# UncertainLab/Enlsip.jl

Hardware: NVIDIA B200
Metric: batched CNLS solves/s (n=6,m=128) (higher is better)
Workload: dtype f64

## Files before the change

### enlsip.jl_b200/csrc/enl_base.h

```cpp
#pragma once
#include <math.h>
#include <stdint.h>
#include <type_traits>

#if defined(__CUDACC__)
#define ENL_FN __device__
#define ENL_INL __device__ __forceinline__
#define ENL_NOINL __device__ __noinline__
#else
#define ENL_FN
#define ENL_INL inline
#define ENL_NOINL
#endif

namespace enl {

#if defined(__CUDA_ARCH__)
ENL_INL double mul_rn(double a, double b) { return __dmul_rn(a, b); }
ENL_INL double add_rn(double a, double b) { return __dadd_rn(a, b); }
ENL_INL double sub_rn(double a, double b) { return __dsub_rn(a, b); }
ENL_INL double fma_rn(double a, double b, double c) { return fma(a, b, c); }
ENL_INL double div_rn(double a, double b) { return __ddiv_rn(a, b); }
ENL_INL double sqrt_rn(double a) { return __dsqrt_rn(a); }
#else
// ... 48 lines not shown
    acc = fma_rn(acc, r, 1.0);
    int k1 = k >> 1;
    int k2 = k - k1;
    double res = mul_rn(mul_rn(acc, pow2i(k1)), pow2i(k2));
    if (x < -745.2) res = 0.0;
    if (x > 709.782712893384) res = INFINITY;
    return (x != x) ? x : res;
}

ENL_INL double det_tanh(double z) {
    double e = det_exp(mul_rn(2.0, z));
    return sub_rn(1.0, div_rn(2.0, add_rn(e, 1.0)));
}

#if defined(__CUDACC__)
template <int G_>
struct DevGroup {
    static constexpr int G = G_;
    unsigned mask;
    int lane;
    __device__ DevGroup() {
        int wl = threadIdx.x & 31;
        lane = wl & (G - 1);
        mask = (G == 32) ? 0xffffffffu : (((1u << G) - 1u) << (wl & ~(G - 1)));
    }
    __device__ __forceinline__ void sync() const {
        if (G > 1) __syncwarp(mask);
    }
    __device__ __forceinline__ double sum(double v) const {
#pragma unroll
        for (int o = G / 2; o > 0; o >>= 1) v += __shfl_xor_sync(mask, v, o, G);
        return v;
    }
    __device__ __forceinline__ double maxv(double v) const {
#pragma unroll
        for (int o = G / 2; o > 0; o >>= 1) v = fmax(v, __shfl_xor_sync(mask, v, o, G));
        return v;
    }
};
#endif

struct HostGroup {
    static constexpr int G = 1;
    int lane = 0;
    void sync() const {}
    double sum(double v) const { return v; }
    double maxv(double v) const { return v; }
};

#if defined(__CUDACC__)
extern __shared__ __align__(16) double enl_smem[];
using vref = int;
ENL_INL vref make_vref(double* p) { return (int)(p - enl_smem); }
ENL_INL vref make_vref(int* p) { return (int)(p - reinterpret_cast<int*>(enl_smem)); }
ENL_INL double& vderef_d(vref o) { return enl_smem[o]; }
ENL_INL int& vderef_i(vref o) { return reinterpret_cast<int*>(enl_smem)[o]; }
#else
using vref = void*;
ENL_INL vref make_vref(double* p) { return p; }
ENL_INL vref make_vref(int* p) { return p; }
#endif

template <int S>
struct SV {
#if defined(__CUDACC__)
    int p;
    ENL_INL double& operator[](int i) const { return enl_smem[p + i * S]; }
#else
    double* p;
    ENL_INL double& operator[](int i) const { return p[i * S]; }
#endif
    ENL_INL SV off(int k) const { return SV{p + k * S}; }
};
template <int S>
struct SI {
#if defined(__CUDACC__)
    int p;
    ENL_INL int& operator[](int i) const { return reinterpret_cast<int*>(enl_smem)[p + i * S]; }
#else
// ... 44 lines not shown
```

### enlsip.jl_b200/csrc/enl_linalg.h

```cpp
#pragma once
#include "enl_base.h"

namespace enl {

#if defined(ENL_HOST_BUILD)
typedef void (*host_dgeqp3_fn)(const int*, const int*, double*, const int*, int*, double*, double*, const int*, int*);
inline host_dgeqp3_fn& host_dgeqp3() { static host_dgeqp3_fn fn = nullptr; return fn; }
inline void host_lapack_qrcp(double* a, int ld, int rows, int cols, double* tau, int* jpvt) {
    static thread_local double work[8192];
    for (int j = 0; j < cols; ++j) jpvt[j] = 0;
    int info = 0;
    const int lwork = 8192;
    host_dgeqp3()(&rows, &cols, a, &ld, jpvt, tau, work, &lwork, &info);
    for (int j = 0; j < cols; ++j) jpvt[j] -= 1;
}
#endif

template <class V>
ENL_NOINL double nrm2_small(V a, int n) {
    double s = 0.0;
#pragma unroll 1
    for (int i = 0; i < n; ++i) s += a[i] * a[i];
    return sqrt(s);
}
// ... 124 lines not shown
        x[i] = s / d;
    }
    return true;
}

template <class V, class V2>
ENL_NOINL bool solve_upperT_small(V R, int ld, int k, V2 x) {
#pragma unroll 1
    for (int i = 0; i < k; ++i) {
        double s = x[i];
#pragma unroll 1
        for (int j = 0; j < i; ++j) s -= R[i * ld + j] * x[j];
        double d = R[i * ld + i];
        if (d == 0.0) return false;
        x[i] = s / d;
    }
    return true;
}

template <class V>
ENL_NOINL int pseudo_rank(V R, int ld, int len, double eps_rank) {
    if (len <= 0 || fabs(R[0]) < eps_rank) return 0;
    double tol = fabs(R[0]) * sqrt((double)len) * eps_rank;
    int r = 1;
#pragma unroll 1
    while (r < len && fabs(R[(r - 1) * ld + (r - 1)]) > tol) ++r;
    return r - ((r == len && fabs(R[(r - 1) * ld + (r - 1)]) > tol) ? 0 : 1);
}

template <class Grp, int G, int MS, int NT>
struct Dist {
    Grp g;

    ENL_NOINL double colsq(DM<G, MS, NT> a, int c, int r0) const {
        double s = 0.0;
#pragma unroll
        for (int sl = 0; sl < MS; ++sl) {
            int row = sl * G + g.lane;
            double v = a.at(sl, c);
            if (row >= r0) s += v * v;
        }
        return g.sum(s);
    }

    template <class V>
    ENL_NOINL void mul_q_right(DM<G, MS, NT> J, int n, V fa, int ld, int k, V tau) const {
#pragma unroll 1
        for (int i = 0; i < k; ++i) {
            double ti = tau[i];
            if (ti == 0.0) continue;
#pragma unroll
            for (int sl = 0; sl < MS; ++sl) {
                double wv = J.at(sl, i);
#pragma unroll 1
                for (int c = i + 1; c < n; ++c) wv += J.at(sl, c) * fa[i * ld + c];
                wv *= ti;
                J.at(sl, i) -= wv;
#pragma unroll 1
                for (int c = i + 1; c < n; ++c) J.at(sl, c) -= wv * fa[i * ld + c];
            }
        }
    }

    template <class V, class VI>
    ENL_NOINL void qrcp(DM<G, MS, NT> a, int M, int ncols, V tau2, VI jpvt, V vn1, V vn2, V Rout, int ldr) const {
#if defined(ENL_HOST_BUILD)
        if (host_dgeqp3() && G == 1 && NT == 1 && M > 0 && ncols > 0) {
            host_lapack_qrcp(&a.at(0, 0), MS, M, ncols, &tau2[0], &jpvt[0]);
            const int kk = imin(M, ncols);
            for (int c = 0; c < ncols; ++c)
                for (int r = 0; r < kk; ++r) Rout[c * ldr + r] = (r <= c) ? a.row(r, c) : 0.0;
            return;
        }
#endif
#pragma unroll 1
        for (int j = 0; j < ncols; ++j) {
            jpvt[j] = j;
            double nj = sqrt(colsq(a, j, 0));
            vn1[j] = nj;
            vn2[j] = nj;
        }
        int k = imin(M, ncols);
#pragma unroll 1
        for (int i = 0; i < k; ++i) {
            int pvt = i;
            double best = vn1[i];
#pragma unroll 1
            for (int j = i + 1; j < ncols; ++j)
                if (vn1[j] > best) { best = vn1[j]; pvt = j; }
            if (pvt != i) {
#pragma unroll
                for (int sl = 0; sl < MS; ++sl) {
                    double tmp = a.at(sl, pvt);
                    a.at(sl, pvt) = a.at(sl, i);
                    a.at(sl, i) = tmp;
                }
                int it = jpvt[pvt]; jpvt[pvt] = jpvt[i]; jpvt[i] = it;
                vn1[pvt] = vn1[i];
                vn2[pvt] = vn2[i];
            }
            g.sync();
            double tau_i = 0.0;
            if (i < M - 1) {
                double alpha = a.row(i, i);
                double xn = sqrt(colsq(a, i, i + 1));
                if (xn != 0.0) {
                    double beta = -sign_of(lapy2(alpha, xn), alpha);
                    tau_i = (beta - alpha) / beta;
                    double sc = 1.0 / (alpha - beta);
                    g.sync();
#pragma unroll
                    for (int sl = 0; sl < MS; ++sl) {
                        int row = sl * G + g.lane;
                        if (row > i) a.at(sl, i) *= sc;
                        else if (row == i) a.at(sl, i) = beta;
                    }
                }
            }
            tau2[i] = tau_i;
            if (i < ncols - 1 && tau_i != 0.0) {
#pragma unroll 1
                for (int c = i + 1; c < ncols; ++c) {
                    double part = 0.0;
#pragma unroll
                    for (int sl = 0; sl < MS; ++sl) {
                        int row = sl * G + g.lane;
                        double vv = (row > i) ? a.at(sl, i) : ((row == i) ? 1.0 : 0.0);
                        part += vv * a.at(sl, c);
                    }
                    double wv = g.sum(part) * tau_i;
#pragma unroll
                    for (int sl = 0; sl < MS; ++sl) {
                        int row = sl * G + g.lane;
                        if (row > i) a.at(sl, c) -= wv * a.at(sl, i);
                        else if (row == i) a.at(sl, c) -= wv;
                    }
                }
            }
            g.sync();
#pragma unroll 1
            for (int j = i + 1; j < ncols; ++j) {
                double v1 = vn1[j];
                if (v1 != 0.0) {
                    double tq = fabs(a.row(i, j)) / v1;
                    double temp = fmax(1.0 - tq * tq, 0.0);
                    double rq = v1 / vn2[j];
                    double temp2 = temp * (rq * rq);
                    if (temp2 <= TOL3Z) {
                        if (i < M - 1) {
                            double nj = sqrt(colsq(a, j, i + 1));
                            vn1[j] = nj;
                            vn2[j] = nj;
                        } else {
                            vn1[j] = 0.0;
                            vn2[j] = 0.0;
                        }
                    } else {
                        vn1[j] = v1 * sqrt(temp);
                    }
                }
            }
        }
        g.sync();
#pragma unroll 1
        for (int c = 0; c < ncols; ++c)
#pragma unroll 1
            for (int r = 0; r < k; ++r) Rout[c * ldr + r] = (r <= c) ? a.row(r, c) : 0.0;
    }

    template <class V>
// ... 13 lines not shown
#pragma unroll
            for (int sl = 0; sl < MS; ++sl) {
                int row = sl * G + g.lane;
                if (row > i) d.at(sl, 0) -= wv * a.at(sl, i);
                else if (row == i) d.at(sl, 0) -= wv;
            }
        }
        g.sync();
    }

    template <class V>
    ENL_NOINL void apply_q_regs(DM<G, MS, NT> a, int k, V tau2, double* v) const {
#pragma unroll 1
        for (int i = k - 1; i >= 0; --i) {
            double ti = tau2[i];
            if (ti == 0.0) continue;
            double part = 0.0;
#pragma unroll
            for (int sl = 0; sl < MS; ++sl) {
                int row = sl * G + g.lane;
                double vv = (row > i) ? a.at(sl, i) : ((row == i) ? 1.0 : 0.0);
                part += vv * v[sl];
            }
            double wv = g.sum(part) * ti;
#pragma unroll
            for (int sl = 0; sl < MS; ++sl) {
                int row = sl * G + g.lane;
                double vv = (row > i) ? a.at(sl, i) : ((row == i) ? 1.0 : 0.0);
                v[sl] -= wv * vv;
            }
        }
    }

    ENL_NOINL double prefix_sq(DM<G, MS, NT> d, int len) const {
        double s = 0.0;
#pragma unroll
        for (int sl = 0; sl < MS; ++sl) {
            int row = sl * G + g.lane;
            double v = d.at(sl, 0);
            if (row < len) s += v * v;
        }
        return g.sum(s);
    }
};

}
```

### enlsip.jl_b200/csrc/enl_solver.h

```cpp
#pragma once
#include "enl_base.h"
#include "enl_linalg.h"
#include "enl_families.h"

namespace enl {

struct Options {
    int max_iter;
    int scaling;
    int jac_mode;
    int second_derivatives;
    double time_limit;
    double eps_abs;
    double eps_rel;
    double eps_x;
    double eps_c;
    double eps_rank;
};

constexpr int MAX_N = 32;
struct Bounds {
    int nlo, nup;
    int lo_idx[MAX_N], up_idx[MAX_N];
    double lo_val[MAX_N], up_val[MAX_N];
// ... 24 lines not shown
    static constexpr size_t smem_bytes() {
        return (size_t)nD * PPC * 8 + (size_t)DCOLS * MS * NT * 8 + (size_t)nI * PPC * 4;
    }
};

struct IterRec {
    int t, rankA, rankJ2, dimA, dimJ2, code, index_del, index_alpha_upp, nb_newton;
    bool restart, add, del;
    double alpha, beta, progress, predicted_reduction, grad_res, speed;
};

struct Outputs {
    double* x;
    double* f;
    int* exit_code;
    int* status;
    int* iters;
    int* nact;
    int* active;
    int* counters;
    double* trace;
    int trace_cap;
};

template <class Fam, class Grp, int NT>
struct Solver {
    static constexpr int G = Grp::G;
    using LY = Layout<Fam, G, NT>;
    static constexpr int N = LY::N, M = LY::M, Q = LY::Q, NNL = LY::NNL, LMAX = LY::LMAX, T = LY::T, PPC = LY::PPC,
                         MS = LY::MS;
    using V = SV<PPC>;
    using VI = SI<PPC>;
    using D = DM<G, MS, NT>;

    V x, xprev, xnew, cx, cnew, A, gradf, w, wnew, K, acx, aA, dsc, FA, tauA, FL, tauL, R2, tau2, lam, b, p, y, Ap, aAp,
        v1c, vn1, vn2, s1, s2, s3, s4, s5, nw;
    VI active, inactive, permA, permL, perm2, posidx;
    D dR, dJ, dF, dD, dY;
    V fs;
    using FCtx = typename Fam::template Ctx<D, V>;
    ENL_INL Grp grp() const { return Grp(); }
    ENL_INL Dist<Grp, G, MS, NT> dst() const { return Dist<Grp, G, MS, NT>(); }
    ENL_INL FCtx fctx() const { return FCtx{dY, fs}; }
    const Options& opt;
    const Bounds& bnd;

    int l, t, k_iter, ndetail, exit_code;
    int n_res, n_cons, n_jres, n_jcons;
    bool threw, hang;
    bool j2_factored;
    IterRec cur, prev;
    double rx_sum, active_cx_sum, f_detail, rdot_x1, cdot_x1, rdot_prev, cdot_prev;
    double jp_r, jp_jp;
    double t_start;

    ENL_FN Solver(double* small, int* ints, double* distbase, int pid, const Options& o, const Bounds& bb)
        : opt(o), bnd(bb) {
#if defined(__CUDACC__)
        int s = (int)(small - enl_smem) + pid;
#else
        double* s = small + pid;
#endif
        auto mk = [&](int off) { return V{s + off * PPC}; };
        x = mk(LY::oX); xprev = mk(LY::oXPREV); xnew = mk(LY::oXNEW); cx = mk(LY::oCX); cnew = mk(LY::oCNEW);
        A = mk(LY::oA); gradf = mk(LY::oGRADF); w = mk(LY::oW); wnew = mk(LY::oWNEW); K = mk(LY::oK);
        acx = mk(LY::oACX); aA = mk(LY::oAA); dsc = mk(LY::oDSC); FA = mk(LY::oFA); tauA = mk(LY::oTAUA);
// ... 6 lines not shown
#else
        int* ii = ints + pid;
#endif
        auto mi = [&](int off) { return VI{ii + off * PPC}; };
        active = mi(LY::iACT); inactive = mi(LY::iINACT); permA = mi(LY::iPERMA); permL = mi(LY::iPERML);
        perm2 = mi(LY::iPERM2); posidx = mi(LY::iPOS);
#if defined(__CUDACC__)
        int grpb = (int)(distbase - enl_smem) + pid * G;
#else
        double* grpb = distbase + pid * G;
#endif
        D all{grpb};
        dR = all; dJ = all.cols(1); dF = dJ; dD = all.cols(1 + N); dY = all.cols(2 + N);
        l = NNL + bnd.nlo + bnd.nup;
    }

    ENL_FN void load_x(V src, double* xv) const {
#pragma unroll
        for (int j = 0; j < N; ++j) xv[j] = src[j];
    }

    ENL_NOINL void eval_point(const double* xv, double* rn, V cout) {
        Fam::template residuals<Grp, MS>(fctx(), grp(), xv, rn);
        double cnl[NNL > 0 ? NNL : 1];
        if (NNL > 0) Fam::template constraints<MS>(fctx(), xv, cnl);
#pragma unroll 1
        for (int i = 0; i < NNL; ++i) cout[i] = cnl[i];
#pragma unroll 1
        for (int j = 0; j < bnd.nlo; ++j) cout[NNL + j] = sub_rn(xv[bnd.lo_idx[j]], bnd.lo_val[j]);
#pragma unroll 1
        for (int j = 0; j < bnd.nup; ++j) cout[NNL + bnd.nlo + j] = sub_rn(bnd.up_val[j], xv[bnd.up_idx[j]]);
    }

    ENL_FN double sumsq_regs(const double* rn) const {
        double s = 0.0;
#pragma unroll
        for (int sl = 0; sl < MS; ++sl) s += rn[sl] * rn[sl];
        return grp().sum(s);
    }

    const double* mat_J = nullptr;
    ENL_NOINL void eval_res_jacobian() {
        if (mat_J) {
#pragma unroll
            for (int sl = 0; sl < MS; ++sl) {
                const int row = sl * G + grp().lane;
#pragma unroll
                for (int j = 0; j < N; ++j) dJ.at(sl, j) = (row < M) ? mat_J[(size_t)j * M + row] : 0.0;
            }
            j2_factored = false;
            grp().sync();
            return;
        }
        double xv[N];
        load_x(x, xv);
        double out[MS * N];
        if (opt.jac_mode == 0) {
            Fam::template jac_residuals<Grp, MS>(fctx(), grp(), xv, out);
        } else {
            double r0[MS], dl[N];
#pragma unroll
            for (int sl = 0; sl < MS; ++sl) r0[sl] = dR.at(sl, 0);
#pragma unroll
            for (int j = 0; j < N; ++j) dl[j] = mul_rn(fmax(fabs(xv[j]), 1.0), SQRT_EPS);
            fd_res(xv, r0, dl, out);
        }
// ... 35 lines not shown
            } else {
                double xf[N], cf[NNL > 0 ? NNL : 1];
#pragma unroll 1
                for (int j = 0; j < N; ++j) {
                    double dj = mul_rn(fmax(fabs(xv[j]), 1.0), SQRT_EPS);
#pragma unroll 1
                    for (int i = 0; i < N; ++i) xf[i] = xv[i];
                    xf[j] = add_rn(xv[j], dj);
                    Fam::template constraints<MS>(fctx(), xf, cf);
#pragma unroll 1
                    for (int i = 0; i < NNL; ++i) An[i * N + j] = div_z(sub_rn(cf[i], cx[i]), dj);
                }
            }
#pragma unroll 1
            for (int i = 0; i < NNL * N; ++i) A[i] = An[i];
        }
    }

    ENL_NOINL void init_bound_rows() {
#pragma unroll 1
        for (int j = 0; j < bnd.nlo; ++j)
#pragma unroll 1
            for (int c = 0; c < N; ++c) A[(NNL + j) * N + c] = (c == bnd.lo_idx[j]) ? 1.0 : 0.0;
#pragma unroll 1
        for (int j = 0; j < bnd.nup; ++j)
#pragma unroll 1
            for (int c = 0; c < N; ++c) A[(NNL + bnd.nlo + j) * N + c] = (c == bnd.up_idx[j]) ? -1.0 : 0.0;
    }

    ENL_NOINL void grad_and_sumsq() {
        double rr[MS];
#pragma unroll
        for (int sl = 0; sl < MS; ++sl) rr[sl] = dR.at(sl, 0);
#pragma unroll 1
        for (int j = 0; j < N; ++j) {
            double s = 0.0;
#pragma unroll
            for (int sl = 0; sl < MS; ++sl) s += dJ.at(sl, j) * rr[sl];
            gradf[j] = grp().sum(s);
        }
        rx_sum = sumsq_regs(rr);
    }

    ENL_FN void ws_remove(int s) {
        int lt = l - t;
        int id = active[s - 1];
        int pos = lt;
#pragma unroll 1
        while (pos > 0 && inactive[pos - 1] > id) { inactive[pos] = inactive[pos - 1]; --pos; }
        inactive[pos] = id;
#pragma unroll 1
        for (int i = s; i <= t - 1; ++i) active[i - 1] = active[i];
        active[t - 1] = 0;
        t -= 1;
    }
    ENL_FN void ws_add(int s) {
        int id = inactive[s - 1];
        int pos = t;
#pragma unroll 1
        while (pos > 0 && active[pos - 1] > id) { active[pos] = active[pos - 1]; --pos; }
        active[pos] = id;
#pragma unroll 1
        for (int i = s; i <= l - t - 1; ++i) inactive[i - 1] = inactive[i];
        inactive[l - t - 1] = 0;
        t += 1;
    }

    ENL_NOINL bool evaluate_violated_constraints(int index_alpha_upp) {
        const double delta = 0.1;
        int cap = imin(l, N);
        bool added = false;
        int swaps = 0;
        if (l > t) {
            int i = 1;
// ... 73 lines not shown
#pragma unroll 1
        for (int i = 0; i < N; ++i) s1[i] = gradf[i];
        apply_qt_small(FA, N, N, t, tauA, s1);
#pragma unroll 1
        for (int i = 0; i < t; ++i) s2[i] = (i < pr) ? s1[i] : 0.0;
        if (!solve_upper_small(FA, N, pr, s2)) threw = true;
        double gr = 0.0;
#pragma unroll 1
        for (int i = pr; i < N; ++i) gr += s1[i] * s1[i];
        cur.grad_res = (N > pr) ? sqrt(gr) : 0.0;
#pragma unroll 1
        for (int j = 0; j < t; ++j) s3[j] = (j < pr) ? -acx[permA[j]] : 0.0;
        if (!solve_upperT_small(FA, N, pr, s3)) threw = true;
        if (!solve_upper_small(FA, N, pr, s3)) threw = true;
#pragma unroll 1
        for (int j = 0; j < t; ++j) lam[permA[j]] = s2[j] + s3[j];
        if (opt.scaling)
#pragma unroll 1
            for (int i = 0; i < t; ++i) lam[i] = lam[i] * dsc[i];
    }

    ENL_NOINL void second_lagrange() {
        int pr = pseudo_rank(FA, N, t, SQRT_EPS);
        double v[MS];
        {
            const int kq = imin(M, N - cur.rankA);
#pragma unroll
            for (int sl = 0; sl < MS; ++sl) {
                int row = sl * G + grp().lane;
                v[sl] = (row >= kq) ? -dD.at(sl, 0) : 0.0;
            }
            dst().apply_q_regs(dF, kq, tau2, v);
        }
#pragma unroll 1
        for (int j = 0; j < t; ++j) {
            double s = 0.0;
#pragma unroll
            for (int sl = 0; sl < MS; ++sl) s += dJ.at(sl, j) * v[sl];
            s1[j] = grp().sum(s);
        }
#pragma unroll 1
        for (int j = pr; j < t; ++j) s1[j] = 0.0;
        if (!solve_upper_small(FA, N, pr, s1)) threw = true;
#pragma unroll 1
        for (int j = 0; j < t; ++j) lam[permA[j]] = s1[j];
        if (opt.scaling)
#pragma unroll 1
            for (int i = 0; i < t; ++i) lam[i] = lam[i] * dsc[i];
    }

    ENL_NOINL int check_constraint_deletion(double grad_res) {
        double lam_max = 1.0;
        if (t > 0) {
            lam_max = 0.0;
#pragma unroll 1
            for (int i = 0; i < t; ++i) lam_max = fmax(lam_max, fabs(lam[i]));
        }
        double sq_rel = SQRT_EPS * lam_max;
        int s = 0;
        if (t > Q) {
            double e = sq_rel;
#pragma unroll 1
            for (int i = Q + 1; i <= t; ++i) {
                double row_i = opt.scaling ? 1.0 / dsc[i - 1] : dsc[i - 1];
                double v = row_i * lam[i - 1];
                if (v <= sq_rel && v <= e) { e = v; s = i; }
            }
            if (grad_res > -e * 10.0) s = 0;
        }
        return s;
    }

    ENL_FN void minmax_lagrangian_mult(double& sigmin, double& lam_abs_max) {
// ... 3 lines not shown
#pragma unroll 1
            for (int i = 0; i < t; ++i) lam_abs_max = fmax(lam_abs_max, fabs(lam[i]));
#pragma unroll 1
            for (int i = Q; i < t; ++i) {
                double rows = opt.scaling ? 1.0 / dsc[i] : dsc[i];
                double li = lam[i];
                if (li * rows <= -SQRT_EPS && li < sigmin) sigmin = li;
            }
        }
    }

    ENL_NOINL void sub_search_direction(int rankA, int dimA, int dimJ2, int code) {
        const int k2 = N - rankA;
        const int kq = imin(M, k2);
        if (code == 1) {
#pragma unroll 1
            for (int j = 0; j < t; ++j) { double v = -acx[permA[j]]; b[j] = v; y[j] = v; }
            if (!solve_upperT_small(FA, N, t, y)) threw = true;
        } else {
#pragma unroll 1
            for (int j = 0; j < t; ++j) s1[j] = -acx[permA[j]];
            apply_qt_small(FL, T, t, t, tauL, s1);
#pragma unroll 1
            for (int j = 0; j < t; ++j) b[j] = s1[j];
            if (dimA > t || dimA < 0) { threw = true; dimA = imax(0, imin(dimA, t)); }
#pragma unroll 1
            for (int j = 0; j < t; ++j) s2[j] = (j < dimA) ? s1[j] : 0.0;
            if (!solve_upper_small(FL, T, dimA, s2)) threw = true;
#pragma unroll 1
            for (int j = 0; j < t; ++j) s3[permL[j]] = s2[j];
#pragma unroll 1
            for (int j = 0; j < rankA; ++j) y[j] = s3[j];
        }
#pragma unroll
        for (int sl = 0; sl < MS; ++sl) {
            double acc = 0.0;
#pragma unroll 1
            for (int c = 0; c < rankA; ++c) acc += dJ.at(sl, c) * y[c];
            dD.at(sl, 0) = -acc - dR.at(sl, 0);
        }
        grp().sync();
        dst().apply_qt(dF, kq, tau2, dD);
        if (dimJ2 > kq || dimJ2 < 0) { threw = true; dimJ2 = imax(0, imin(dimJ2, kq)); }
#pragma unroll 1
        for (int j = 0; j < dimJ2; ++j) s2[j] = dD.row(j, 0);
        if (!solve_upper_small(R2, N, dimJ2, s2)) threw = true;
#pragma unroll 1
        for (int j = 0; j < k2; ++j) y[rankA + perm2[j]] = (j < dimJ2) ? s2[j] : 0.0;
#pragma unroll 1
        for (int j = 0; j < N; ++j) p[j] = y[j];
        apply_q_small(FA, N, N, t, tauA, p);
    }

    ENL_NOINL void gn_search_direction(int rankA) {
        int code = (rankA == t) ? 1 : -1;
        dst().mul_q_right(dJ, N, FA, N, t, tauA);
        const int k2 = N - rankA;
        dF = dJ.cols(rankA);
        grp().sync();
        dst().qrcp(dF, M, k2, tau2, perm2, vn1, vn2, R2, N);
        j2_factored = true;
        int rankJ2 = pseudo_rank(R2, N, imin(M, k2), opt.eps_rank);
        sub_search_direction(rankA, rankA, rankJ2, code);
        cur.rankA = rankA;
        cur.rankJ2 = rankJ2;
        cur.dimA = rankA;
        cur.dimJ2 = rankJ2;
    }

    ENL_NOINL void update_working_set() {
        factor_A();
        first_lagrange();
        int s = check_constraint_deletion(cur.grad_res);
        if (s != 0) {
            cur.index_del = 0;
            cur.del = false;
            if (opt.scaling) {
#pragma unroll 1
                for (int i = 0; i < t; ++i) {
                    int id = active[i] - 1;
#pragma unroll 1
                    for (int c = 0; c < N; ++c) aA[i * N + c] = A[id * N + c] * dsc[i];
                }
                factor_A();
            }
        }
#pragma unroll 1
        for (int pass = 0; pass < 2; ++pass) {
            int rankA = pseudo_rank(FA, N, t, opt.eps_rank);
            factor_L11();
            gn_search_direction(rankA);
            if (pass == 0 && t == rankA && cur.rankJ2 == imin(M, N - rankA)) {
                second_lagrange();
// ... 102 lines not shown
        double prev_alpha = prev.alpha;
        int pdA;
        const int k2 = N - rankA;
        const int kq = imin(M, k2);
        if (rankA <= 0) {
            dimA = 0;
            pdA = 0;
#pragma unroll
            for (int sl = 0; sl < MS; ++sl) dD.at(sl, 0) = -dR.at(sl, 0);
        } else {
            pdA = abs(prev.dimA) + t - prev.t;
            if (pdA > t) { threw = true; pdA = t; }
            double sb = 0.0, sa = 0.0;
#pragma unroll 1
            for (int j = 0; j < t; ++j) {
                sb += b[j] * b[j];
                if (j < pdA) sa += b[j] * b[j];
            }
            double nrm_b = sqrt(sb), nrm_b_asprev = sqrt(sa);
            double cprog = cdot_prev - active_cx_sum;
            dimA = determine_solving_dim(pdA, rankA, nrm_b, cprog, nrm_b_asprev, FL, T, b, prev_alpha, restart);
            if (dimA > t || rankA - dimA < 0) { threw = true; dimA = imin(dimA, rankA); }
#pragma unroll 1
            for (int j = 0; j < rankA; ++j) s2[j] = (j < dimA) ? b[j] : 0.0;
            if (!solve_upper_small(FL, T, dimA, s2)) threw = true;
#pragma unroll 1
            for (int i = 0; i < rankA; ++i) {
                double acc = 0.0;
#pragma unroll 1
                for (int j = 0; j < rankA; ++j)
                    if (permL[j] == i) acc += s2[j];
                s3[i] = acc;
            }
#pragma unroll
            for (int sl = 0; sl < MS; ++sl) {
                double acc = 0.0;
#pragma unroll 1
                for (int c = 0; c < rankA; ++c) acc += dJ.at(sl, c) * s3[c];
                dD.at(sl, 0) = -(dR.at(sl, 0) + acc);
            }
        }
        grp().sync();
        if (rankJ2 > 0) dst().apply_qt(dF, kq, tau2, dD);
        int pdJ = abs(prev.dimJ2) + prev.t - t;
        if (pdJ > M) { threw = true; pdJ = M; }
        double nrm_d_asprev = sqrt(dst().prefix_sq(dD, pdJ));
        double nrm_d = sqrt(dst().prefix_sq(dD, M));
        double rprog = rdot_prev - rx_sum;
        if (rankJ2 > M) { threw = true; }
#pragma unroll 1
        for (int j = 0; j < rankJ2 && j < M; ++j) s2[j] = dD.row(j, 0);
        dimJ2 = determine_solving_dim(pdJ, rankJ2, nrm_d, rprog, nrm_d_asprev, R2, N, s2, prev_alpha, restart);
        if (!restart && prev_alpha >= alpha_low) {
            dimA = imax(dimA, pdA);
            dimJ2 = imax(dimJ2, pdJ);
        }
    }

    ENL_NOINL int check_gn_direction(double b1nrm, double d1nrm, double d1nrm_as_km1, double dnrm, double active_c_sum,
                                  int rankA, bool restart, bool added, bool deleted, double& beta_k) {
        const double delta = 1e-1;
        const double c1 = 0.5, c2 = 0.1, c3 = 4.0, c4 = 10.0, c5 = 0.05;
        beta_k = sqrt(d1nrm * d1nrm + b1nrm * b1nrm);
        int method = 1;
        bool newton_or_restart = (prev.code == 2) || restart;
        bool first_iter = (k_iter == 0);
        bool submin_prev = prev.code == -1;
        bool add_or_del = added || deleted;
        bool conv_lower = beta_k < c1 * prev.beta;
        bool progress_not_close = (prev.progress > c2 * prev.predicted_reduction) && (dnrm <= c3 * beta_k);
        if (newton_or_restart || (!first_iter && (submin_prev || !(add_or_del || conv_lower || progress_not_close)))) {
            method = -1;
            double nonlin_k = sqrt(d1nrm * d1nrm + active_c_sum);
            double nonlin_km1 = sqrt(d1nrm_as_km1 * d1nrm_as_km1 + active_c_sum);
            bool to_reduce = false;
            if (Q < t) {
                bool any_ge = false, any_neg = false;
#pragma unroll 1
                for (int i = Q; i < t; ++i) {
                    double rows = opt.scaling ? 1.0 / dsc[i] : dsc[i];
// ... 88 lines not shown
                double sr = 0.0;
#pragma unroll
                for (int sl = 0; sl < MS; ++sl) sr += fa[sl] * rr[sl];
                sr = grp().sum(sr) / (4 * ej * ek);
                double sc = 0.0;
#pragma unroll 1
                for (int i = 0; i < t; ++i) sc += cacc[active[i] - 1] * lam[i];
                sc = sc / (4.0 * ek * ej);
                Gm[j * N + kk] = sr - sc;
                Gm[kk * N + j] = sr - sc;
            }
#pragma unroll 1
        for (int c = 0; c < N; ++c) apply_qt_small(FA, N, N, t, tauA, Gm.off(c * N));
#pragma unroll 1
        for (int r = 0; r < N; ++r) {
#pragma unroll 1
            for (int c = 0; c < N; ++c) s1[c] = Gm[c * N + r];
            apply_qt_small(FA, N, N, t, tauA, s1);
#pragma unroll 1
            for (int c = 0; c < N; ++c) Em[c * N + r] = s1[c];
        }
        if (t > rankA) {
            if (t != N) { threw = true; return true; }
#pragma unroll 1
            for (int c = 0; c < N; ++c)
#pragma unroll 1
                for (int r = 0; r < N; ++r) Gm[c * N + r] = Em[permL[c] * N + permL[r]];
#pragma unroll 1
            for (int i = 0; i < N * N; ++i) Em[i] = Gm[i];
        }
        const int k2 = N - rankA;
#pragma unroll 1
        for (int a = 0; a < k2; ++a) {
#pragma unroll 1
            for (int c = 0; c < N; ++c) {
                double s = 0.0;
#pragma unroll
                for (int sl = 0; sl < MS; ++sl) s += dJ.at(sl, rankA + a) * dJ.at(sl, c);
                s1[c] = grp().sum(s);
            }
            double sjr = 0.0;
#pragma unroll
            for (int sl = 0; sl < MS; ++sl) sjr += dJ.at(sl, rankA + a) * rr[sl];
            sjr = grp().sum(sjr);
            double dacc = 0.0;
#pragma unroll 1
            for (int c = 0; c < rankA; ++c) dacc += (Em[c * N + (rankA + a)] + s1[c]) * y[c];
            s2[a] = -dacc - sjr;
#pragma unroll 1
            for (int c2 = 0; c2 < k2; ++c2) Wm[c2 * N + a] = Em[(rankA + c2) * N + (rankA + a)] + s1[rankA + c2];
        }
#pragma unroll 1
        for (int a = 0; a < k2; ++a)
#pragma unroll 1
            for (int c = a; c < k2; ++c) {
                double v = (Wm[c * N + a] + Wm[a * N + c]) * 0.5;
                Gm[c * N + a] = v;
            }
#pragma unroll 1
        for (int j = 0; j < k2; ++j) {
            double ajj = Gm[j * N + j];
#pragma unroll 1
            for (int i = 0; i < j; ++i) ajj -= Gm[j * N + i] * Gm[j * N + i];
            if (!(ajj > 0.0)) {
#pragma unroll 1
                for (int i = 0; i < N; ++i) p[i] = 0.0;
#pragma unroll 1
                for (int i = 0; i < N; ++i) y[i] = 0.0;
                return true;
            }
            ajj = sqrt(ajj);
            Gm[j * N + j] = ajj;
#pragma unroll 1
            for (int c = j + 1; c < k2; ++c) {
                double v = Gm[c * N + j];
#pragma unroll 1
                for (int i = 0; i < j; ++i) v -= Gm[j * N + i] * Gm[c * N + i];
                Gm[c * N + j] = v / ajj;
            }
        }
        solve_upperT_small(Gm, N, k2, s2);
        solve_upper_small(Gm, N, k2, s2);
#pragma unroll 1
        for (int a = 0; a < k2; ++a) y[rankA + a] = s2[a];
#pragma unroll 1
        for (int j = 0; j < N; ++j) p[j] = y[j];
        apply_q_small(FA, N, N, t, tauA, p);
        return false;
    }

    ENL_NOINL int search_direction_analys() {
        const int rankA = cur.rankA, rankJ2 = cur.rankJ2;
        double sb = 0.0;
#pragma unroll 1
        for (int j = 0; j < cur.dimA; ++j) sb += b[j] * b[j];
        double nrm_b1_gn = sqrt(sb);
        double nrm_d_gn = sqrt(dst().prefix_sq(dD, M));
        double nrm_d1_gn = sqrt(dst().prefix_sq(dD, cur.dimJ2));
        int pd = prev.dimJ2 + prev.t - t - 1;
        if (pd > M) { threw = true; pd = M; }
        double nrm_d1_asprev = sqrt(dst().prefix_sq(dD, pd));
        bool restart = cur.restart;
        int error_code = 0;
        double beta;
        int method = check_gn_direction(nrm_b1_gn, nrm_d1_gn, nrm_d1_asprev, nrm_d_gn, active_cx_sum, rankA, restart,
                                        cur.add, cur.del, beta);
        int dimA = rankA, dimJ2 = rankJ2;
        if (method == -1) {
#pragma unroll 1
            for (int j = 0; j < t; ++j) s1[j] = -acx[permA[j]];
            apply_qt_small(FL, T, t, t, tauL, s1);
#pragma unroll 1
            for (int j = 0; j < t; ++j) b[j] = s1[j];
            choose_subspace_dimensions(rankA, rankJ2, restart, dimA, dimJ2);
            if (!threw) sub_search_direction(rankA, dimA, dimJ2, -1);
            if (dimA == rankA && dimJ2 == rankJ2) method = 1;
        } else if (method == 2) {
            if (opt.second_derivatives) {
                bool nerr = newton_search_direction(rankA);
                dimA = -t;
                dimJ2 = t - N;
                cur.nb_newton += 1;
                if (nerr) error_code = -3;
            } else {
                error_code = -4;
            }
        }
        cur.dimA = dimA;
        cur.dimJ2 = dimJ2;
        cur.code = method;
        cur.speed = beta / prev.beta;
        cur.beta = beta;
        return error_code;
    }
// ... 251 lines not shown
                double phi = acos(arg);
                double tt = (cc <= 0) ? 2 * sqrt(-bb / 3) : -2 * sqrt(-bb / 3);
                const double PI = 3.141592653589793;
                double b1 = tt * cos(phi / 3) - a1 / 3;
                double b2 = tt * cos((phi + 2 * PI) / 3) - a1 / 3;
                double b3 = tt * cos((phi + 4 * PI) / 3) - a1 / 3;
                double tmp;
                if (b1 > b2) { tmp = b1; b1 = b2; b2 = tmp; }
                if (b2 > b3) { tmp = b2; b2 = b3; b3 = tmp; }
                if (b1 > b2) { tmp = b1; b1 = b2; b2 = tmp; }
                if (x_min <= b2) { alpha_hat = b1; beta_hat = b3; } else { alpha_hat = b3; beta_hat = b1; }
                have_beta = true;
            } else {
                if (d != d) { threw = true; alpha_hat = beta_hat = x_min; return; }
                double sd = sqrt(d);
                alpha_hat = cbrt(-cc / 2 + sd) + cbrt(-cc / 2 - sd) - a1 / 3;
            }
        } else {
            alpha_hat = newton_raphson(x_min, Dm, ds, dds);
        }
        if (d >= 0) { beta_hat = alpha_hat; have_beta = true; }
        if (!have_beta) threw = true;
    }

    ENL_NOINL void minrm(const double* jp, const double* rn, double alpha_k, double x_min, double amin, double amax,
                      double& a_hat, double& s_a, double& b_hat, double& s_b) {
        double d00 = 0, d01 = 0, d02 = 0, d11 = 0, d12 = 0, d22 = 0;
#pragma unroll
        for (int sl = 0; sl < MS; ++sl) {
            double v0 = dR.at(sl, 0), v1 = jp[sl];
            double v2 = ((rn[sl] - v0) / alpha_k - v1) / alpha_k;
            d00 += v0 * v0; d01 += v0 * v1; d02 += v0 * v2; d11 += v1 * v1; d12 += v1 * v2; d22 += v2 * v2;
        }
        d00 = grp().sum(d00); d01 = grp().sum(d01); d02 = grp().sum(d02); d11 = grp().sum(d11); d12 = grp().sum(d12); d22 = grp().sum(d22);
#pragma unroll 1
        for (int i = 0; i < l; ++i) s1[i] = 0.0;
#pragma unroll 1
        for (int i = 0; i < t; ++i) s1[active[i] - 1] = 1.0;
#pragma unroll 1
        for (int kk = 0; kk < l; ++kk) {
            const bool act = s1[kk] != 0.0;
            if (!act && cx[kk] > 0 && cnew[kk] > 0) continue;
            double sw = sqrt(wnew[kk]);
            double v0, vb;
            if (act) { v0 = sw * cx[kk]; vb = sw * cnew[kk]; }
            else { v0 = (cx[kk] > 0) ? 0.0 : sw * cx[kk]; vb = (cnew[kk] > 0) ? 0.0 : sw * cnew[kk]; }
            double v1 = v1c[kk];
            double v2 = (div_z(vb - v0, alpha_k) - v1) / alpha_k;
            d00 += v0 * v0; d01 += v0 * v1; d02 += v0 * v2; d11 += v1 * v1; d12 += v1 * v2; d22 += v2 * v2;
        }
        Quartic s;
        s.len = 5;
        s.c[0] = 0.5 * d00; s.c[1] = d01; s.c[2] = d02 + 0.5 * d11; s.c[3] = d12; s.c[4] = 0.5 * d22;
        s.chop();
        Quartic ds = s.derivative();
        Quartic dds = ds.derivative();
        parameters_rm(d12, d22, x_min, ds, dds, a_hat, b_hat);
        double a_old = a_hat;
        auto bounds = [&](double a) { if (a != a) return a; a = fmin(a, amax); a = fmax(a, amin); return a; };
        a_hat = bounds(a_hat);
        s_a = s(a_hat);
        if (a_old == b_hat) { b_hat = a_hat; s_b = s(a_hat); }
        else { b_hat = bounds(b_hat); s_b = s(b_hat); }
    }

    ENL_FN static bool check_reduction(double psi_alpha, double psi_k, double approx_k, double eta, double diff_psi) {
        if (psi_alpha - approx_k >= eta * diff_psi) return !((psi_alpha - psi_k < eta * diff_psi) && (psi_k > 0.2 * psi_alpha));
// ... 97 lines not shown

    ENL_FN double upper_bound_steplength(int index_del, int& index_alpha_upp) {
        double alpha_upper = INFINITY;
        index_alpha_upp = 0;
#pragma unroll 1
        for (int i = 0; i < l - t; ++i) {
            int j = inactive[i];
            if (j != index_del) {
                double gp = Ap[j - 1];
                double a_j = -cx[j - 1] / gp;
                if (cx[j - 1] > 0 && gp < 0 && a_j < alpha_upper) { alpha_upper = a_j; index_alpha_upp = j; }
            }
        }
        return fmin(3.0, alpha_upper);
    }

    ENL_NOINL double compute_steplength(int& Psi_error, double* rfin, bool& have_final) {
        double jp[MS];
        if (j2_factored) {
            const int rankA = cur.rankA, k2 = N - cur.rankA, kq = imin(M, N - cur.rankA);
#pragma unroll 1
            for (int i = 0; i < kq; ++i) {
                double acc = 0.0;
#pragma unroll 1
                for (int j = i; j < k2; ++j) acc += R2[j * N + i] * y[rankA + perm2[j]];
                s1[i] = acc;
            }
#pragma unroll
            for (int sl = 0; sl < MS; ++sl) {
                int row = sl * G + grp().lane;
                jp[sl] = (row < kq) ? s1[row < kq ? row : 0] : 0.0;
            }
            dst().apply_q_regs(dF, kq, tau2, jp);
#pragma unroll
            for (int sl = 0; sl < MS; ++sl) {
                double acc = 0.0;
#pragma unroll 1
                for (int c = 0; c < rankA; ++c) acc += dJ.at(sl, c) * y[c];
                jp[sl] += acc;
            }
        } else {
#pragma unroll
            for (int sl = 0; sl < MS; ++sl) {
                double acc = 0.0;
#pragma unroll 1
                for (int c = 0; c < N; ++c) acc += dJ.at(sl, c) * y[c];
                jp[sl] = acc;
            }
        }
        {
            double a = 0.0, bq = 0.0;
#pragma unroll
            for (int sl = 0; sl < MS; ++sl) { a += jp[sl] * dR.at(sl, 0); bq += jp[sl] * jp[sl]; }
            jp_r = grp().sum(a);
            jp_jp = grp().sum(bq);
        }
#pragma unroll 1
        for (int i = 0; i < NNL; ++i) {
            double acc = 0.0;
#pragma unroll 1
            for (int c = 0; c < N; ++c) acc += A[i * N + c] * p[c];
            Ap[i] = acc;
        }
#pragma unroll 1
        for (int j = 0; j < bnd.nlo; ++j) Ap[NNL + j] = p[bnd.lo_idx[j]];
#pragma unroll 1
        for (int j = 0; j < bnd.nup; ++j) Ap[NNL + bnd.nlo + j] = -p[bnd.up_idx[j]];
#pragma unroll 1
        for (int i = 0; i < t; ++i) {
            double acc = 0.0;
#pragma unroll 1
            for (int c = 0; c < N; ++c) acc += aA[i * N + c] * p[c];
            aAp[i] = opt.scaling ? acc / dsc[i] : acc;
        }
        Psi_error = 0;
        have_final = false;
        double alpha;
        if (cur.code != 2) {
            double dpsi0 = penalty_weight_update(jp, cur.dimA);
            double pen = 0.0;
#pragma unroll 1
            for (int i = 0; i < t; ++i) { int kk = active[i] - 1; pen += wnew[kk] * (cx[kk] * cx[kk]); }
            double psi0 = 0.5 * (rx_sum + pen);
            if (dpsi0 >= 0) {
                alpha = 1.0;
                Psi_error = -1;
                cur.index_alpha_upp = 0;
            } else {
// ... 41 lines not shown

    ENL_NOINL int check_termination(int error_code, bool time_up, double sigma_min, double lam_abs_max, int Psi_error) {
        int ec = 0;
        double pn = 0.0;
#pragma unroll 1
        for (int j = 0; j < N; ++j) pn += p[j] * p[j];
        double alfnoi = EPS / (sqrt(pn) + EPS);
        bool preliminary = !(cur.restart || (cur.code == -1 && alfnoi <= 0.25));
        double xd = 0.0, xn2 = 0.0;
#pragma unroll 1
        for (int j = 0; j < N; ++j) { double dd = xprev[j] - xnew[j]; xd += dd * dd; xn2 += xnew[j] * xnew[j]; }
        double x_diff = sqrt(xd);
        if (preliminary) {
            double ca = 0.0, gn = 0.0;
#pragma unroll 1
            for (int i = 0; i < t; ++i) ca += acx[i] * acx[i];
#pragma unroll 1
            for (int j = 0; j < N; ++j) gn += gradf[j] * gradf[j];
            bool necessary = (!cur.del) && (sqrt(ca) < opt.eps_c) && (cur.grad_res < sqrt(opt.eps_rel) * (1 + sqrt(gn)));
            if (l - t > 0) {
                bool allpos = true;
#pragma unroll 1
                for (int i = 0; i < l - t; ++i)
                    if (!(cx[inactive[i] - 1] > 0)) allpos = false;
                necessary = necessary && allpos;
            }
            if (t > Q) {
                double factor = (t == 1) ? (1 + rx_sum) : lam_abs_max;
                necessary = necessary && (sigma_min >= opt.eps_rel * factor);
            }
            if (necessary) {
                int dj = cur.dimJ2;
                if (dj > M) { threw = true; dj = M; }
                double d1 = dst().prefix_sq(dD, dj);
                if (d1 <= rx_sum * opt.eps_rel * opt.eps_rel) ec += 10000;
                if (rx_sum <= opt.eps_abs * opt.eps_abs) ec += 2000;
                if (x_diff < opt.eps_x * sqrt(xn2)) ec += 300;
                if (alfnoi > 0.25) ec += 40;
                if (ec > 0 && l - t > 0) {
                    int feas = 1;
#pragma unroll 1
                    for (int i = 0; i < l - t; ++i)
                        if (cx[inactive[i] - 1] <= 0.0) { feas = -1; break; }
                    ec *= feas;
                }
            }
        }
        if (ec == 0) {
            double an = 0.0;
#pragma unroll 1
            for (int c = 0; c < N; ++c) {
                double acc = 0.0;
#pragma unroll 1
                for (int i = 0; i < t; ++i) acc += aA[i * N + c] * acx[i];
                an += acc * acc;
            }
            double Atcx_nrm = sqrt(an);
            double aps = 0.0;
#pragma unroll 1
            for (int i = 0; i < t; ++i) { double wi = wnew[active[i] - 1]; aps += wi * wi; }
            if (k_iter >= opt.max_iter) ec = -2;
            else if (error_code >= -5 && error_code <= -3) ec = error_code;
            else if (cur.nb_newton > 5) ec = -9;
            else if (Psi_error == -1) ec = -6;
            else if (x_diff <= 10.0 * opt.eps_x && Atcx_nrm <= 10.0 * opt.eps_c && aps >= 1.0) ec = -10;
            else if (time_up) ec = -11;
        }
        return ec;
// ... 269 lines not shown
```

Baseline: 2.023 million.

## Batch warp-shuffle reductions across multiple dot products and restructure J-matrix loops

```diff
diff --git a/enlsip.jl_b200/csrc/enl_base.h b/enlsip.jl_b200/csrc/enl_base.h
--- a/enlsip.jl_b200/csrc/enl_base.h
+++ b/enlsip.jl_b200/csrc/enl_base.h
@@ -104,6 +104,13 @@
         for (int o = G / 2; o > 0; o >>= 1) v += __shfl_xor_sync(mask, v, o, G);
         return v;
     }
+    template <int K>
+    __device__ __forceinline__ void sums(double (&v)[K]) const {
+#pragma unroll
+        for (int o = G / 2; o > 0; o >>= 1)
+#pragma unroll
+            for (int k = 0; k < K; ++k) v[k] += __shfl_xor_sync(mask, v[k], o, G);
+    }
     __device__ __forceinline__ double maxv(double v) const {
 #pragma unroll
         for (int o = G / 2; o > 0; o >>= 1) v = fmax(v, __shfl_xor_sync(mask, v, o, G));
@@ -117,6 +124,8 @@
     int lane = 0;
     void sync() const {}
     double sum(double v) const { return v; }
+    template <int K>
+    void sums(double (&)[K]) const {}
     double maxv(double v) const { return v; }
 };
 
diff --git a/enlsip.jl_b200/csrc/enl_linalg.h b/enlsip.jl_b200/csrc/enl_linalg.h
--- a/enlsip.jl_b200/csrc/enl_linalg.h
+++ b/enlsip.jl_b200/csrc/enl_linalg.h
@@ -180,6 +180,25 @@
 struct Dist {
     Grp g;
 
+    template <int K, class XF, class YF, class OUT>
+    ENL_INL void dots(int n, XF xf, YF yf, OUT out) const {
+#pragma unroll 1
+        for (int j0 = 0; j0 < n; j0 += K) {
+            double s[K];
+#pragma unroll
+            for (int q = 0; q < K; ++q) {
+                s[q] = 0.0;
+                if (j0 + q < n)
+#pragma unroll
+                    for (int sl = 0; sl < MS; ++sl) s[q] += xf(sl, j0 + q) * yf(sl, j0 + q);
+            }
+            g.sums(s);
+#pragma unroll
+            for (int q = 0; q < K; ++q)
+                if (j0 + q < n) out(j0 + q, s[q]);
+        }
+    }
+
     ENL_NOINL double colsq(DM<G, MS, NT> a, int c, int r0) const {
         double s = 0.0;
 #pragma unroll
@@ -197,20 +216,30 @@
         for (int i = 0; i < k; ++i) {
             double ti = tau[i];
             if (ti == 0.0) continue;
+            double wv[MS];
+#pragma unroll
+            for (int sl = 0; sl < MS; ++sl) wv[sl] = J.at(sl, i);
+#pragma unroll 1
+            for (int c = i + 1; c < n; ++c) {
+                const double f = fa[i * ld + c];
+#pragma unroll
+                for (int sl = 0; sl < MS; ++sl) wv[sl] += J.at(sl, c) * f;
+            }
 #pragma unroll
             for (int sl = 0; sl < MS; ++sl) {
-                double wv = J.at(sl, i);
-#pragma unroll 1
-                for (int c = i + 1; c < n; ++c) wv += J.at(sl, c) * fa[i * ld + c];
-                wv *= ti;
-                J.at(sl, i) -= wv;
-#pragma unroll 1
-                for (int c = i + 1; c < n; ++c) J.at(sl, c) -= wv * fa[i * ld + c];
-            }
-        }
-    }
-
-    template <class V, class VI>
+                wv[sl] *= ti;
+                J.at(sl, i) -= wv[sl];
+            }
+#pragma unroll 1
+            for (int c = i + 1; c < n; ++c) {
+                const double f = fa[i * ld + c];
+#pragma unroll
+                for (int sl = 0; sl < MS; ++sl) J.at(sl, c) -= wv[sl] * f;
+            }
+        }
+    }
+
+    template <int KB, class V, class VI>
     ENL_NOINL void qrcp(DM<G, MS, NT> a, int M, int ncols, V tau2, VI jpvt, V vn1, V vn2, V Rout, int ldr) const {
 #if defined(ENL_HOST_BUILD)
         if (host_dgeqp3() && G == 1 && NT == 1 && M > 0 && ncols > 0) {
@@ -221,12 +250,14 @@
             return;
         }
 #endif
-#pragma unroll 1
-        for (int j = 0; j < ncols; ++j) {
-            jpvt[j] = j;
-            double nj = sqrt(colsq(a, j, 0));
-            vn1[j] = nj;
-            vn2[j] = nj;
+        {
+            auto col = [&](int sl, int j) { return a.at(sl, j); };
+            dots<KB>(ncols, col, col, [&](int j, double s) {
+                jpvt[j] = j;
+                double nj = sqrt(s);
+                vn1[j] = nj;
+                vn2[j] = nj;
+            });
         }
         int k = imin(M, ncols);
 #pragma unroll 1
@@ -267,23 +298,23 @@
             }
             tau2[i] = tau_i;
             if (i < ncols - 1 && tau_i != 0.0) {
-#pragma unroll 1
-                for (int c = i + 1; c < ncols; ++c) {
-                    double part = 0.0;
+                double vv[MS];
+#pragma unroll
+                for (int sl = 0; sl < MS; ++sl) {
+                    int row = sl * G + g.lane;
+                    vv[sl] = (row > i) ? a.at(sl, i) : ((row == i) ? 1.0 : 0.0);
+                }
+                DM<G, MS, NT> trail = a.cols(i + 1);
+                dots<(KB > 1) ? KB - 1 : 1>(ncols - 1 - i, [&](int sl, int) { return vv[sl]; },
+                                            [&](int sl, int q) { return trail.at(sl, q); }, [&](int q, double s) {
+                    double wv = s * tau_i;
 #pragma unroll
                     for (int sl = 0; sl < MS; ++sl) {
-                        int row = sl * G + g.lane;
-                        double vv = (row > i) ? a.at(sl, i) : ((row == i) ? 1.0 : 0.0);
-                        part += vv * a.at(sl, c);
+                        double& e = trail.at(sl, q);
+                        double upd = e - wv * vv[sl];
+                        e = (sl * G + g.lane >= i) ? upd : e;
                     }
-                    double wv = g.sum(part) * tau_i;
-#pragma unroll
-                    for (int sl = 0; sl < MS; ++sl) {
-                        int row = sl * G + g.lane;
-                        if (row > i) a.at(sl, c) -= wv * a.at(sl, i);
-                        else if (row == i) a.at(sl, c) -= wv;
-                    }
-                }
+                });
             }
             g.sync();
 #pragma unroll 1
@@ -363,15 +394,19 @@
         }
     }
 
-    ENL_NOINL double prefix_sq(DM<G, MS, NT> d, int len) const {
-        double s = 0.0;
-#pragma unroll
-        for (int sl = 0; sl < MS; ++sl) {
-            int row = sl * G + g.lane;
-            double v = d.at(sl, 0);
-            if (row < len) s += v * v;
-        }
-        return g.sum(s);
+    template <int K>
+    ENL_INL void prefix_sq(DM<G, MS, NT> d, const int (&len)[K], double (&s)[K]) const {
+        double v[MS];
+#pragma unroll
+        for (int sl = 0; sl < MS; ++sl) v[sl] = d.at(sl, 0);
+#pragma unroll
+        for (int k = 0; k < K; ++k) {
+            s[k] = 0.0;
+#pragma unroll
+            for (int sl = 0; sl < MS; ++sl)
+                if (sl * G + g.lane < len[k]) s[k] += v[sl] * v[sl];
+        }
+        g.sums(s);
     }
 };
 
diff --git a/enlsip.jl_b200/csrc/enl_solver.h b/enlsip.jl_b200/csrc/enl_solver.h
--- a/enlsip.jl_b200/csrc/enl_solver.h
+++ b/enlsip.jl_b200/csrc/enl_solver.h
@@ -80,6 +80,7 @@
     using V = SV<PPC>;
     using VI = SI<PPC>;
     using D = DM<G, MS, NT>;
+    static constexpr int KB_N = (N < 8) ? N : 8, KB_N1 = (N + 1 < 8) ? N + 1 : 8;
 
     V x, xprev, xnew, cx, cnew, A, gradf, w, wnew, K, acx, aA, dsc, FA, tauA, FL, tauL, R2, tau2, lam, b, p, y, Ap, aAp,
         v1c, vn1, vn2, s1, s2, s3, s4, s5, nw;
@@ -152,6 +153,17 @@
         for (int j = 0; j < bnd.nup; ++j) cout[NNL + bnd.nlo + j] = sub_rn(bnd.up_val[j], xv[bnd.up_idx[j]]);
     }
 
+    ENL_INL void jmul(int ncols, V v, double* acc) const {
+#pragma unroll
+        for (int sl = 0; sl < MS; ++sl) acc[sl] = 0.0;
+#pragma unroll 1
+        for (int c = 0; c < ncols; ++c) {
+            const double vc = v[c];
+#pragma unroll
+            for (int sl = 0; sl < MS; ++sl) acc[sl] += dJ.at(sl, c) * vc;
+        }
+    }
+
     ENL_FN double sumsq_regs(const double* rn) const {
         double s = 0.0;
 #pragma unroll
@@ -253,14 +265,9 @@
         double rr[MS];
 #pragma unroll
         for (int sl = 0; sl < MS; ++sl) rr[sl] = dR.at(sl, 0);
-#pragma unroll 1
-        for (int j = 0; j < N; ++j) {
-            double s = 0.0;
-#pragma unroll
-            for (int sl = 0; sl < MS; ++sl) s += dJ.at(sl, j) * rr[sl];
-            gradf[j] = grp().sum(s);
-        }
-        rx_sum = sumsq_regs(rr);
+        dst().template dots<KB_N1>(N + 1, [&](int sl, int j) { return (j < N) ? dJ.at(sl, j) : rr[sl]; },
+                                   [&](int sl, int) { return rr[sl]; },
+                                   [&](int j, double s) { if (j < N) gradf[j] = s; else rx_sum = s; });
     }
 
     ENL_FN void ws_remove(int s) {
@@ -400,13 +407,8 @@
             }
             dst().apply_q_regs(dF, kq, tau2, v);
         }
-#pragma unroll 1
-        for (int j = 0; j < t; ++j) {
-            double s = 0.0;
-#pragma unroll
-            for (int sl = 0; sl < MS; ++sl) s += dJ.at(sl, j) * v[sl];
-            s1[j] = grp().sum(s);
-        }
+        dst().template dots<KB_N>(t, [&](int sl, int j) { return dJ.at(sl, j); }, [&](int sl, int) { return v[sl]; },
+                                  [&](int j, double s) { s1[j] = s; });
 #pragma unroll 1
         for (int j = pr; j < t; ++j) s1[j] = 0.0;
         if (!solve_upper_small(FA, N, pr, s1)) threw = true;
@@ -476,12 +478,11 @@
 #pragma unroll 1
             for (int j = 0; j < rankA; ++j) y[j] = s3[j];
         }
-#pragma unroll
-        for (int sl = 0; sl < MS; ++sl) {
-            double acc = 0.0;
-#pragma unroll 1
-            for (int c = 0; c < rankA; ++c) acc += dJ.at(sl, c) * y[c];
-            dD.at(sl, 0) = -acc - dR.at(sl, 0);
+        {
+            double acc[MS];
+            jmul(rankA, y, acc);
+#pragma unroll
+            for (int sl = 0; sl < MS; ++sl) dD.at(sl, 0) = -acc[sl] - dR.at(sl, 0);
         }
         grp().sync();
         dst().apply_qt(dF, kq, tau2, dD);
@@ -502,7 +503,7 @@
         const int k2 = N - rankA;
         dF = dJ.cols(rankA);
         grp().sync();
-        dst().qrcp(dF, M, k2, tau2, perm2, vn1, vn2, R2, N);
+        dst().template qrcp<KB_N>(dF, M, k2, tau2, perm2, vn1, vn2, R2, N);
         j2_factored = true;
         int rankJ2 = pseudo_rank(R2, N, imin(M, k2), opt.eps_rank);
         sub_search_direction(rankA, rankA, rankJ2, code);
@@ -671,20 +672,20 @@
                     if (permL[j] == i) acc += s2[j];
                 s3[i] = acc;
             }
-#pragma unroll
-            for (int sl = 0; sl < MS; ++sl) {
-                double acc = 0.0;
-#pragma unroll 1
-                for (int c = 0; c < rankA; ++c) acc += dJ.at(sl, c) * s3[c];
-                dD.at(sl, 0) = -(dR.at(sl, 0) + acc);
-            }
+            double acc[MS];
+            jmul(rankA, s3, acc);
+#pragma unroll
+            for (int sl = 0; sl < MS; ++sl) dD.at(sl, 0) = -(dR.at(sl, 0) + acc[sl]);
         }
         grp().sync();
         if (rankJ2 > 0) dst().apply_qt(dF, kq, tau2, dD);
         int pdJ = abs(prev.dimJ2) + prev.t - t;
         if (pdJ > M) { threw = true; pdJ = M; }
-        double nrm_d_asprev = sqrt(dst().prefix_sq(dD, pdJ));
-        double nrm_d = sqrt(dst().prefix_sq(dD, M));
+        const int lens[2] = {pdJ, M};
+        double sq[2];
+        dst().prefix_sq(dD, lens, sq);
+        double nrm_d_asprev = sqrt(sq[0]);
+        double nrm_d = sqrt(sq[1]);
         double rprog = rdot_prev - rx_sum;
         if (rankJ2 > M) { threw = true; }
 #pragma unroll 1
@@ -839,17 +840,10 @@
         const int k2 = N - rankA;
 #pragma unroll 1
         for (int a = 0; a < k2; ++a) {
-#pragma unroll 1
-            for (int c = 0; c < N; ++c) {
-                double s = 0.0;
-#pragma unroll
-                for (int sl = 0; sl < MS; ++sl) s += dJ.at(sl, rankA + a) * dJ.at(sl, c);
-                s1[c] = grp().sum(s);
-            }
             double sjr = 0.0;
-#pragma unroll
-            for (int sl = 0; sl < MS; ++sl) sjr += dJ.at(sl, rankA + a) * rr[sl];
-            sjr = grp().sum(sjr);
+            dst().template dots<KB_N1>(N + 1, [&](int sl, int) { return dJ.at(sl, rankA + a); },
+                                       [&](int sl, int c) { return (c < N) ? dJ.at(sl, c) : rr[sl]; },
+                                       [&](int c, double s) { if (c < N) s1[c] = s; else sjr = s; });
             double dacc = 0.0;
 #pragma unroll 1
             for (int c = 0; c < rankA; ++c) dacc += (Em[c * N + (rankA + a)] + s1[c]) * y[c];
@@ -902,11 +896,14 @@
 #pragma unroll 1
         for (int j = 0; j < cur.dimA; ++j) sb += b[j] * b[j];
         double nrm_b1_gn = sqrt(sb);
-        double nrm_d_gn = sqrt(dst().prefix_sq(dD, M));
-        double nrm_d1_gn = sqrt(dst().prefix_sq(dD, cur.dimJ2));
         int pd = prev.dimJ2 + prev.t - t - 1;
         if (pd > M) { threw = true; pd = M; }
-        double nrm_d1_asprev = sqrt(dst().prefix_sq(dD, pd));
+        const int lens[3] = {M, cur.dimJ2, pd};
+        double sq[3];
+        dst().prefix_sq(dD, lens, sq);
+        double nrm_d_gn = sqrt(sq[0]);
+        double nrm_d1_gn = sqrt(sq[1]);
+        double nrm_d1_asprev = sqrt(sq[2]);
         bool restart = cur.restart;
         int error_code = 0;
         double beta;
@@ -1224,7 +1221,11 @@
             double v2 = ((rn[sl] - v0) / alpha_k - v1) / alpha_k;
             d00 += v0 * v0; d01 += v0 * v1; d02 += v0 * v2; d11 += v1 * v1; d12 += v1 * v2; d22 += v2 * v2;
         }
-        d00 = grp().sum(d00); d01 = grp().sum(d01); d02 = grp().sum(d02); d11 = grp().sum(d11); d12 = grp().sum(d12); d22 = grp().sum(d22);
+        {
+            double d[6] = {d00, d01, d02, d11, d12, d22};
+            grp().sums(d);
+            d00 = d[0]; d01 = d[1]; d02 = d[2]; d11 = d[3]; d12 = d[4]; d22 = d[5];
+        }
 #pragma unroll 1
         for (int i = 0; i < l; ++i) s1[i] = 0.0;
 #pragma unroll 1
@@ -1388,28 +1389,20 @@
                 jp[sl] = (row < kq) ? s1[row < kq ? row : 0] : 0.0;
             }
             dst().apply_q_regs(dF, kq, tau2, jp);
-#pragma unroll
-            for (int sl = 0; sl < MS; ++sl) {
-                double acc = 0.0;
-#pragma unroll 1
-                for (int c = 0; c < rankA; ++c) acc += dJ.at(sl, c) * y[c];
-                jp[sl] += acc;
-            }
+            double acc[MS];
+            jmul(rankA, y, acc);
+#pragma unroll
+            for (int sl = 0; sl < MS; ++sl) jp[sl] += acc[sl];
         } else {
-#pragma unroll
-            for (int sl = 0; sl < MS; ++sl) {
-                double acc = 0.0;
-#pragma unroll 1
-                for (int c = 0; c < N; ++c) acc += dJ.at(sl, c) * y[c];
-                jp[sl] = acc;
-            }
+            jmul(N, y, jp);
         }
         {
-            double a = 0.0, bq = 0.0;
-#pragma unroll
-            for (int sl = 0; sl < MS; ++sl) { a += jp[sl] * dR.at(sl, 0); bq += jp[sl] * jp[sl]; }
-            jp_r = grp().sum(a);
-            jp_jp = grp().sum(bq);
+            double d[2] = {0.0, 0.0};
+#pragma unroll
+            for (int sl = 0; sl < MS; ++sl) { d[0] += jp[sl] * dR.at(sl, 0); d[1] += jp[sl] * jp[sl]; }
+            grp().sums(d);
+            jp_r = d[0];
+            jp_jp = d[1];
         }
 #pragma unroll 1
         for (int i = 0; i < NNL; ++i) {
@@ -1517,8 +1510,10 @@
             if (necessary) {
                 int dj = cur.dimJ2;
                 if (dj > M) { threw = true; dj = M; }
-                double d1 = dst().prefix_sq(dD, dj);
-                if (d1 <= rx_sum * opt.eps_rel * opt.eps_rel) ec += 10000;
+                const int lens[1] = {dj};
+                double d1[1];
+                dst().prefix_sq(dD, lens, d1);
+                if (d1[0] <= rx_sum * opt.eps_rel * opt.eps_rel) ec += 10000;
                 if (rx_sum <= opt.eps_abs * opt.eps_abs) ec += 2000;
                 if (x_diff < opt.eps_x * sqrt(xn2)) ec += 300;
                 if (alfnoi > 0.25) ec += 40;
```

Result: no change. 2.031 million, median of 6 (+0.4%).
